# nnaisense/evotorch

Hardware: NVIDIA H100
Metric: PGPE generations/sec at popsize=1Mxdim=10k (Rastrigin, fp32) (higher is better)
Workload: dtype f32

## Files before the change

evotorch_b200/csrc/evok_grad.cu:

```cuda
#include <dlfcn.h>

#include <atomic>
#include <cstdlib>

#include "evok_common.cuh"

#ifndef EVOK_GRAD_TMA_DEFAULT
#define EVOK_GRAD_TMA_DEFAULT 1
#endif

namespace evok {

constexpr int kGradThreads = 256;
constexpr int kGradUnroll = 4;
constexpr int kGradMinBlocks = 4;
constexpr int kGradCtasPerSm = 4;
constexpr int kMaxResidentCtas = kNumSMs * 8;

template <int VEC>
struct VecF;
template <>
struct VecF<4> {
  float v[4];
};
template <>
struct VecF<1> {
  float v[1];
};

template <int VEC>
__device__ __forceinline__ VecF<VEC> load_row(const float* p) {
  VecF<VEC> r;
  if (VEC == 4) {
    const float4 t = ld_stream4(p);
    r.v[0] = t.x; r.v[1] = t.y; r.v[2] = t.z; r.v[3] = t.w;
  } else {
    r.v[0] = ld_stream1(p);
  }
  return r;
}

struct GradItems {
  int64_t x, w, mu, sigma, partial;
};

struct SepWeights {
  const float* q;
  int active;
  float* wsum_partial;
};

constexpr int kEpsRead = 0, kEpsRegen = 1, kEpsRebuild = 2;

__device__ __forceinline__ void grad_coeffs(int form, float s, float& c1, float& c0) {
  if (form == EVOK_GRAD_EXP) {
    c1 = __fdiv_rn(1.0f, s * s);
    c0 = 1.0f;
  } else if (form == EVOK_GRAD_MOMENTS) {
    c1 = 1.0f;
    c0 = 0.0f;
  } else {
    c1 = __fdiv_rn(1.0f, s);
    c0 = s;
  }
}

template <bool SYM, bool SEPW = false>
__device__ __forceinline__ void row_weights(const float* __restrict__ w, int64_t r, float& a, float& b, int64_t D = 0,
                                            const SepWeights* sepw = nullptr) {
  if (SEPW) {
    const float aw = __ldg(w + r);
    a = fmaxf(aw, 0.0f);
    b = (sepw->active && aw < 0.0f) ? __fdiv_rn((float)D * aw, __ldg(sepw->q + r)) : aw;
  } else if (SYM) {
    const float wp = __ldg(w + 2 * r), wm = __ldg(w + 2 * r + 1);
    a = 0.5f * (wp - wm);
    b = 0.5f * (wp + wm);
  } else {
    a = b = __ldg(w + r);
  }
}

__device__ __forceinline__ void accumulate(float a, float b, float e, float c1, float c0, float& s1, float& s2) {
  s1 = fmaf(a, e, s1);
  s2 = fmaf(b, fmaf(e * e, c1, -c0), s2);
}

template <int VEC, bool TAIL = true>
__device__ __forceinline__ void store_partial(float* partial, int64_t chunk, int64_t D, int64_t col, const float* s1, const float* s2) {
  float* p1 = partial + (chunk * 2 + 0) * D + col;
  float* p2 = partial + (chunk * 2 + 1) * D + col;
#pragma unroll
  for (int c = 0; c < VEC; ++c) {
    if (!TAIL || col + c < D) {
      p1[c] = s1[c];
      p2[c] = s2[c];
    }
  }
}

template <int VEC, int TX, bool SYM, int EPS, bool SEPW = false>
__global__ void __launch_bounds__(kGradThreads, kGradMinBlocks)
    grad_partial_kernel(int form, const float* __restrict__ X, int64_t ldx, const float* __restrict__ w, const float* __restrict__ mu,
                        const float* __restrict__ sigma, int64_t n_units, int64_t D, int64_t units_per_chunk, uint64_t unit0,
                        const __grid_constant__ PhiloxKey key, const uint32_t* __restrict__ stream_off, float* __restrict__ partial,
                        const __grid_constant__ GradItems items, const __grid_constant__ SepWeights sepw) {
  static_assert(!SEPW || (EPS == kEpsRegen && !SYM), "the CMA-ES weight mode regenerates non-symmetric rows");
  constexpr int TY = kGradThreads / TX;
  if (gridDim.z > 1) {
    const int64_t item = blockIdx.z;
    X += item * items.x;
    w += item * items.w;
    mu += item * items.mu;
    sigma += item * items.sigma;
    partial += item * items.partial;
  }
  const uint32_t sw = key.stream_lo + ((EPS != kEpsRead && stream_off) ? __ldg(stream_off) : 0u) + (EPS == kEpsRebuild ? (uint32_t)blockIdx.z : 0u);
  const int tx = threadIdx.x % TX, ty = threadIdx.x / TX;
  const int64_t col = ((int64_t)blockIdx.x * TX + tx) * VEC;
  const bool active = col < D;

  float m[VEC], c1[VEC], c0[VEC], sg[VEC];
#pragma unroll
  for (int c = 0; c < VEC; ++c) {
    const bool ok = active && (col + c < D) && !SEPW;
    const float s = ok ? __ldg(sigma + col + c) : 1.0f;
    m[c] = ok ? __ldg(mu + col + c) : 0.0f;
    sg[c] = s;
    grad_coeffs(form, s, c1[c], c0[c]);
  }

  float s1[VEC], s2[VEC];
#pragma unroll
  for (int c = 0; c < VEC; ++c) s1[c] = s2[c] = 0.0f;

  const int64_t r_begin = (int64_t)blockIdx.y * units_per_chunk;
  const int64_t r_end = min(n_units, r_begin + units_per_chunk);
  float wb = 0.0f;

  for (int64_t r0 = r_begin + ty; r0 < r_end; r0 += (int64_t)TY * kGradUnroll) {
    float a[kGradUnroll], b[kGradUnroll];
    bool need[kGradUnroll];
    VecF<VEC> x[kGradUnroll];
#pragma unroll
    for (int u = 0; u < kGradUnroll; ++u) {
      const int64_t r = r0 + (int64_t)u * TY;
      a[u] = b[u] = 0.0f;
      if (r < r_end) {
        row_weights<SYM, SEPW>(w, r, a[u], b[u], D, &sepw);
        if (SEPW) wb += b[u];
      }
      need[u] = active && (a[u] != 0.0f || b[u] != 0.0f);
    }
#pragma unroll
    for (int u = 0; u < kGradUnroll; ++u) {
      const int64_t r = r0 + (int64_t)u * TY;
      if (need[u]) {
        if (EPS != kEpsRead) {
          if (VEC == 4) {
            normals4(key, sw, unit0 + (uint64_t)r, (uint32_t)(col >> 2), x[u].v);
          } else {
            float z[4];
            normals4(key, sw, unit0 + (uint64_t)r, (uint32_t)(col >> 2), z);
            x[u].v[0] = z[col & 3];
          }
        } else {
          x[u] = load_row<VEC>(X + (SYM ? 2 * r : r) * ldx + col);
        }
      }
    }
#pragma unroll
    for (int u = 0; u < kGradUnroll; ++u) {
      if (need[u]) {
#pragma unroll
        for (int c = 0; c < VEC; ++c) {
          const float e = EPS == kEpsRegen ? sg[c] * x[u].v[c] : EPS == kEpsRebuild ? fmaf(sg[c], x[u].v[c], m[c]) - m[c] : x[u].v[c] - m[c];
          accumulate(a[u], b[u], e, c1[c], c0[c], s1[c], s2[c]);
        }
      }
    }
  }

  __shared__ float red[TY > 1 ? TY : 1][TX][2 * VEC];
  if (TY > 1) {
#pragma unroll
    for (int c = 0; c < VEC; ++c) {
      red[ty][tx][c] = s1[c];
      red[ty][tx][VEC + c] = s2[c];
    }
    __syncthreads();
    if (ty == 0) {
#pragma unroll
      for (int c = 0; c < VEC; ++c) {
        float t1 = red[0][tx][c], t2 = red[0][tx][VEC + c];
        for (int y = 1; y < TY; ++y) {
          t1 += red[y][tx][c];
          t2 += red[y][tx][VEC + c];
        }
        s1[c] = t1;
        s2[c] = t2;
      }
    }
  }
  if (ty == 0 && active) store_partial<VEC>(partial, blockIdx.y, D, col, s1, s2);
  if (SEPW && blockIdx.x == 0) {
    __shared__ float wred[TY];
    if (tx == 0) wred[ty] = wb;
    __syncthreads();
    if (threadIdx.x == 0) {
      float t = wred[0];
      for (int y = 1; y < TY; ++y) t += wred[y];
      sepw.wsum_partial[blockIdx.y] = t;
    }
  }
}

__device__ __forceinline__ void sum_chunks(const float* __restrict__ partial, int n_chunks, int64_t D, int64_t j, float& t1, float& t2) {
  t1 = 0.0f;
  t2 = 0.0f;
  for (int c = 0; c < n_chunks; ++c) {
    t1 += partial[((int64_t)c * 2 + 0) * D + j];
    t2 += partial[((int64_t)c * 2 + 1) * D + j];
  }
}

template <bool WSUM = false>
__global__ void __launch_bounds__(256) grad_finalize_kernel(const float* __restrict__ partial, int n_chunks, int64_t D, float scale_mu,
                                                            float scale_sigma, float* __restrict__ out_mu, float* __restrict__ out_sigma,
                                                            int64_t item_stride_partial = 0, const float* __restrict__ wsum_partial = nullptr,
                                                            float* __restrict__ wsum_out = nullptr) {
  const int64_t j = (int64_t)blockIdx.x * blockDim.x + threadIdx.x;
  if (WSUM && j == 0) {
    float t = 0.0f;
    for (int c = 0; c < n_chunks; ++c) t += wsum_partial[c];
    *wsum_out = t;
  }
  if (j >= D) return;
  partial += (int64_t)blockIdx.y * item_stride_partial;
  out_mu += (int64_t)blockIdx.y * D;
  out_sigma += (int64_t)blockIdx.y * D;
  float t1, t2;
  sum_chunks(partial, n_chunks, D, j, t1, t2);
  out_mu[j] = t1 * scale_mu;
  out_sigma[j] = t2 * scale_sigma;
}

struct GradPush {
  PeerSink sink;
  const unsigned long long* epoch;
  unsigned int* done;
};

__global__ void __launch_bounds__(256) grad_finalize_push_kernel(const float* __restrict__ partial, int n_chunks, int64_t D, float scale_mu,
                                                                 float scale_sigma, const __grid_constant__ PeerSink sink,
                                                                 const unsigned long long* epoch, unsigned int* done) {
  const int64_t j = (int64_t)blockIdx.x * blockDim.x + threadIdx.x;
  if (j < D) {
    float t1, t2;
    sum_chunks(partial, n_chunks, D, j, t1, t2);
    t1 *= scale_mu;
    t2 *= scale_sigma;
    for (int p = 0; p < sink.world; ++p) {
      float* slot = static_cast<float*>(sink.data[p]) + (int64_t)sink.rank * 2 * D;
      slot[j] = t1;
      slot[D + j] = t2;
    }
  }
  peer_signal_tail(sink, epoch, done);
}

#ifndef EVOK_GRAD_TMA_ROWS
#define EVOK_GRAD_TMA_ROWS 4
#endif
#ifndef EVOK_GRAD_TMA_STAGES
#define EVOK_GRAD_TMA_STAGES 4
#endif
#ifndef EVOK_GRAD_TMA_CTAS_PER_SM
#define EVOK_GRAD_TMA_CTAS_PER_SM 3
#endif
constexpr int kTmaRows = EVOK_GRAD_TMA_ROWS;
constexpr int kTmaStages = EVOK_GRAD_TMA_STAGES;
constexpr int kTmaCols = 1024;
constexpr int kTmaConsumers = 256;
constexpr int kTmaThreads = kTmaConsumers + 32;
constexpr size_t kTmaSmemBytes = (size_t)kTmaStages * kTmaRows * kTmaCols * sizeof(float) + 2 * kTmaStages * sizeof(uint64_t) + 128;

__device__ __forceinline__ uint32_t smem_u32(const void* p) { return (uint32_t)__cvta_generic_to_shared(p); }
__device__ __forceinline__ void mbar_init(uint64_t* bar, uint32_t count) {
  asm volatile("mbarrier.init.shared::cta.b64 [%0], %1;" ::"r"(smem_u32(bar)), "r"(count) : "memory");
}
__device__ __forceinline__ void mbar_expect_tx(uint64_t* bar, uint32_t bytes) {
  asm volatile("mbarrier.arrive.expect_tx.shared::cta.b64 _, [%0], %1;" ::"r"(smem_u32(bar)), "r"(bytes) : "memory");
}
__device__ __forceinline__ void mbar_arrive(uint64_t* bar) {
  asm volatile("mbarrier.arrive.shared::cta.b64 _, [%0];" ::"r"(smem_u32(bar)) : "memory");
}
__device__ __forceinline__ void mbar_wait(uint64_t* bar, uint32_t parity) {
  asm volatile(
      "{\n"
      ".reg .pred P1;\n"
      "LAB_WAIT:\n"
      "mbarrier.try_wait.parity.shared::cta.b64 P1, [%0], %1;\n"
      "@P1 bra DONE;\n"
      "bra LAB_WAIT;\n"
      "DONE:\n"
      "}" ::"r"(smem_u32(bar)), "r"(parity) : "memory");
}
__device__ __forceinline__ void bulk_load(void* dst_smem, const void* src_gmem, uint32_t bytes, uint64_t* bar) {
  asm volatile("cp.async.bulk.shared::cluster.global.mbarrier::complete_tx::bytes [%0], [%1], %2, [%3];" ::"r"(smem_u32(dst_smem)),
               "l"(src_gmem), "r"(bytes), "r"(smem_u32(bar))
               : "memory");
}

constexpr int kSplitPeriod = 16;
__device__ __forceinline__ uint32_t rebuilt_mask(int split) {
  uint32_t m = 0;
#pragma unroll
  for (int k = 0; k < kSplitPeriod; ++k)
    if ((k + 1) * split / kSplitPeriod > k * split / kSplitPeriod) m |= 1u << k;
  return m;
}
__device__ __forceinline__ bool group_rebuilt(uint32_t mask, int64_t g) { return (mask >> ((int)g & (kSplitPeriod - 1))) & 1u; }

template <bool SYM>
__global__ void __launch_bounds__(kTmaThreads, EVOK_GRAD_TMA_CTAS_PER_SM)
    grad_partial_tma_kernel(int form, const float* __restrict__ X, int64_t ldx, const float* __restrict__ w, const float* __restrict__ mu,
                            const float* __restrict__ sigma, int64_t n_units, int64_t D, int64_t units_per_chunk, int split, uint64_t unit0,
                            const __grid_constant__ PhiloxKey key, const uint32_t* __restrict__ stream_off, float* __restrict__ partial) {
  extern __shared__ __align__(128) unsigned char smem_raw[];
  float* tiles = reinterpret_cast<float*>(smem_raw);
  uint64_t* full = reinterpret_cast<uint64_t*>(smem_raw + (size_t)kTmaStages * kTmaRows * kTmaCols * sizeof(float));
  uint64_t* empty = full + kTmaStages;

  const int tid = threadIdx.x, warp = tid >> 5, lane = tid & 31;
  const int64_t col0 = (int64_t)blockIdx.x * kTmaCols;
  const int64_t width = min((int64_t)kTmaCols, D - col0);
  const int64_t r_begin = (int64_t)blockIdx.y * units_per_chunk;
  const int64_t r_end = min(n_units, r_begin + units_per_chunk);
  const int64_t n_rows = r_end - r_begin;
  const int64_t n_groups = (n_rows + kTmaRows - 1) / kTmaRows;
  const int64_t row_stride = (SYM ? 2 : 1) * ldx;
  const uint32_t mask = rebuilt_mask(split);

  if (tid == 0) {
    for (int s = 0; s < kTmaStages; ++s) {
      mbar_init(&full[s], 1);
      mbar_init(&empty[s], kTmaConsumers / 32);
    }
    asm volatile("fence.mbarrier_init.release.cluster;" ::: "memory");
  }
  __syncthreads();

  if (warp == kTmaConsumers / 32) {
    if (lane == 0) {
      const uint32_t row_bytes = (uint32_t)(width * sizeof(float));
      int64_t t = 0;
      for (int64_t g = 0; g < n_groups; ++g) {
        if (group_rebuilt(mask, g)) continue;
        const int s = (int)(t % kTmaStages);
        const uint32_t use = (uint32_t)(t / kTmaStages);
        ++t;
        if (use > 0) mbar_wait(&empty[s], (use - 1) & 1);
        const int64_t r0 = r_begin + g * kTmaRows;
        const int rows = (int)min((int64_t)kTmaRows, r_end - r0);
        mbar_expect_tx(&full[s], rows * row_bytes);
        float* dst = tiles + (size_t)s * kTmaRows * kTmaCols;
        for (int i = 0; i < rows; ++i) bulk_load(dst + (size_t)i * kTmaCols, X + (r0 + i) * row_stride + col0, row_bytes, &full[s]);
      }
    }
    return;
  }

  const int64_t col = col0 + (int64_t)tid * 4;
  const bool active = col < D;
  const uint32_t sw = key.stream_lo + (stream_off ? __ldg(stream_off) : 0u);
  const int frm = SYM ? EVOK_GRAD_SYMMETRIC : form;
  float m[4], sg[4], c1[4], c0[4];
#pragma unroll
  for (int c = 0; c < 4; ++c) {
    sg[c] = active ? __ldg(sigma + col + c) : 1.0f;
    m[c] = active ? __ldg(mu + col + c) : 0.0f;
    grad_coeffs(frm, sg[c], c1[c], c0[c]);
  }
  float s1[4] = {0.f, 0.f, 0.f, 0.f}, s2[4] = {0.f, 0.f, 0.f, 0.f};

  int64_t t = 0;
  for (int64_t g = 0; g < n_groups; ++g) {
    const int64_t r0 = r_begin + g * kTmaRows;
    const int rows = (int)min((int64_t)kTmaRows, r_end - r0);
    float a[kTmaRows], b[kTmaRows];
    bool need[kTmaRows];
#pragma unroll
    for (int i = 0; i < kTmaRows; ++i) {
      a[i] = b[i] = 0.0f;
      if (i < rows) row_weights<SYM>(w, r0 + i, a[i], b[i]);
      need[i] = a[i] != 0.0f || b[i] != 0.0f;
    }
    if (group_rebuilt(mask, g)) {
      if (active) {
        float x[kTmaRows][4];
#pragma unroll
        for (int i = 0; i < kTmaRows; ++i) {
          float z[4];
          normals4(key, sw, unit0 + (uint64_t)(r0 + i), (uint32_t)(col >> 2), z);
#pragma unroll
          for (int c = 0; c < 4; ++c) x[i][c] = fmaf(sg[c], z[c], m[c]);
        }
#pragma unroll
        for (int i = 0; i < kTmaRows; ++i) {
          if (need[i]) {
#pragma unroll
            for (int c = 0; c < 4; ++c) accumulate(a[i], b[i], x[i][c] - m[c], c1[c], c0[c], s1[c], s2[c]);
          }
        }
      }
      continue;
    }
    const int s = (int)(t % kTmaStages);
    const uint32_t use = (uint32_t)(t / kTmaStages);
    ++t;
    mbar_wait(&full[s], use & 1);
    const float4* tile = reinterpret_cast<const float4*>(tiles + (size_t)s * kTmaRows * kTmaCols) + tid;
    if (active) {
      float4 v4[kTmaRows];
#pragma unroll
      for (int i = 0; i < kTmaRows; ++i) v4[i] = tile[(size_t)i * (kTmaCols / 4)];
#pragma unroll
      for (int i = 0; i < kTmaRows; ++i) {
        if (need[i]) {
          const float4 v = v4[i];
          const float x[4] = {v.x, v.y, v.z, v.w};
#pragma unroll
          for (int c = 0; c < 4; ++c) accumulate(a[i], b[i], x[c] - m[c], c1[c], c0[c], s1[c], s2[c]);
        }
      }
    }
    __syncwarp();
    if (lane == 0) mbar_arrive(&empty[s]);
  }
  if (active) store_partial<4, false>(partial, blockIdx.y, D, col, s1, s2);
}

constexpr int kAutoSplitCapped = 2;
constexpr int kAutoSplitFull = 5;
constexpr int64_t kFullPowerMilliwatts = 550000;

static int auto_split_for_power(int64_t milliwatts) { return milliwatts >= kFullPowerMilliwatts ? kAutoSplitFull : kAutoSplitCapped; }

static int64_t enforced_power_limit_mw(int device) {
  char bus_id[32];
  if (cudaDeviceGetPCIBusId(bus_id, (int)sizeof(bus_id), device) != cudaSuccess) {
    cudaGetLastError();
    return -1;
  }
  void* nvml = dlopen("libnvidia-ml.so.1", RTLD_NOW | RTLD_LOCAL);
  if (!nvml) return -1;
  using init_t = int (*)();
  using by_bus_t = int (*)(const char*, void**);
  using limit_t = int (*)(void*, unsigned int*);
  const auto init = reinterpret_cast<init_t>(dlsym(nvml, "nvmlInit_v2"));
  const auto shutdown = reinterpret_cast<init_t>(dlsym(nvml, "nvmlShutdown"));
  const auto by_bus = reinterpret_cast<by_bus_t>(dlsym(nvml, "nvmlDeviceGetHandleByPciBusId_v2"));
  const auto limit = reinterpret_cast<limit_t>(dlsym(nvml, "nvmlDeviceGetEnforcedPowerLimit"));
  int64_t mw = -1;
  if (init && shutdown && by_bus && limit && init() == 0) {
    void* handle = nullptr;
    unsigned int v = 0;
    if (by_bus(bus_id, &handle) == 0 && limit(handle, &v) == 0) mw = v;
    shutdown();
  }
  dlclose(nvml);
  return mw;
}

static int device_auto_split() {
  constexpr int kMaxDevices = 64;
  static std::atomic<int> resolved[kMaxDevices];
  int device = 0;
  if (cudaGetDevice(&device) != cudaSuccess || device < 0 || device >= kMaxDevices) {
    cudaGetLastError();
    return kAutoSplitCapped;
  }
  int s = resolved[device].load(std::memory_order_relaxed);
  if (s == 0) {
    s = auto_split_for_power(enforced_power_limit_mw(device)) + 1;
    resolved[device].store(s, std::memory_order_relaxed);
  }
  return s - 1;
}


struct GradCall {
  GradCall(int form, int eps, const float* w, const float* mu, const float* sigma, int64_t n_rows, int64_t D, float scale_mu, float scale_sigma,
           float* out_mu, float* out_sigma, void* ws, size_t ws_bytes, void* stream)
      : form(form), eps(eps), w(w), mu(mu), sigma(sigma), n_rows(n_rows), D(D), scale_mu(scale_mu), scale_sigma(scale_sigma), out_mu(out_mu),
        out_sigma(out_sigma), ws(ws), ws_bytes(ws_bytes), st((cudaStream_t)stream) {}
  int form;
  int eps;
  const float* w;
  const float* mu;
  const float* sigma;
  int64_t n_rows, D;
  float scale_mu, scale_sigma;
  float* out_mu;
  float* out_sigma;
  void* ws;
  size_t ws_bytes;
  cudaStream_t st;
  const float* X = nullptr;
  int64_t ldx = 0;
  int64_t row0 = 0;
  PhiloxKey key{};
  const uint32_t* stream_off = nullptr;
  bool batched = false;
  int64_t n_items = 1;
  GradItems items{0, 0, 0, 0, 0};
  int split = 0;
  SepWeights sepw{nullptr, 0, nullptr};
  float* wsum = nullptr;
  const GradPush* push = nullptr;
};

static bool is_sym(const GradCall& c) { return c.form == EVOK_GRAD_SYMMETRIC; }

struct GradPlan {
  bool tma;
  int vec, tx, n_coltiles, n_chunks;
  int64_t n_units, units_per_chunk;
};

static void set_chunks(GradPlan& p, int64_t chunks) {
  if (chunks < 1) chunks = 1;
  if (chunks > 65535) chunks = 65535;
  p.units_per_chunk = (p.n_units + chunks - 1) / chunks;
  p.n_chunks = (int)((p.n_units + p.units_per_chunk - 1) / p.units_per_chunk);
}

static bool tma_enabled() {
  const char* env = getenv("EVOK_GRAD_TMA");
  return env ? atoi(env) != 0 : EVOK_GRAD_TMA_DEFAULT != 0;
}

static GradPlan plan_grad(const GradCall& c) {
  GradPlan p{};
  p.n_units = is_sym(c) ? c.n_rows / 2 : c.n_rows;
  const bool vec_ok = c.eps == kEpsRegen || (c.D % 4 == 0 && (c.eps == kEpsRebuild || (c.ldx % 4 == 0 && aligned16(c.X) && c.items.x % 4 == 0)) &&
                                             c.items.mu % 4 == 0 && c.items.sigma % 4 == 0);
  p.vec = vec_ok ? 4 : 1;
  p.tma = !c.batched && c.eps == kEpsRead && vec_ok && c.form != EVOK_GRAD_MOMENTS && c.D >= 512 && p.n_units >= 4096 && tma_enabled();
  if (p.tma) {
    p.n_coltiles = (int)((c.D + kTmaCols - 1) / kTmaCols);
    set_chunks(p, (int64_t)kNumSMs * EVOK_GRAD_TMA_CTAS_PER_SM / p.n_coltiles);
    return p;
  }
  const int64_t col_threads = (c.D + p.vec - 1) / p.vec;
  p.tx = 32;
  while (p.tx < kGradThreads && p.tx < col_threads) p.tx <<= 1;
  p.n_coltiles = (int)((col_threads + p.tx - 1) / p.tx);
  const int ty = kGradThreads / p.tx;
  int64_t chunks = (int64_t)kNumSMs * kGradCtasPerSm / p.n_coltiles;
  const int64_t max_useful = (p.n_units + (int64_t)ty * kGradUnroll * 16 - 1) / ((int64_t)ty * kGradUnroll * 16);
  set_chunks(p, chunks < max_useful ? chunks : max_useful);
  chunks = ((int64_t)kNumSMs * kGradCtasPerSm + (int64_t)p.n_coltiles * c.n_items - 1) / ((int64_t)p.n_coltiles * c.n_items);
  if (chunks < p.n_chunks) set_chunks(p, chunks);
  if (c.eps == kEpsRebuild && !vec_ok) {
    p.vec = 4;
    p.n_coltiles = (int)(((c.D + 3) / 4 + p.tx - 1) / p.tx);
  }
  return p;
}

using PartialKernel = void (*)(int, const float*, int64_t, const float*, const float*, const float*, int64_t, int64_t, int64_t, uint64_t,
                               PhiloxKey, const uint32_t*, float*, GradItems, SepWeights);
#define EVOK_GRAD_TXS(VEC, SYM, EPS, SEPW)                                                                             \
  {                                                                                                                    \
    grad_partial_kernel<VEC, 32, SYM, EPS, SEPW>, grad_partial_kernel<VEC, 64, SYM, EPS, SEPW>,                        \
        grad_partial_kernel<VEC, 128, SYM, EPS, SEPW>, grad_partial_kernel<VEC, 256, SYM, EPS, SEPW>                   \
  }
static const PartialKernel kPartialKernels[9][4] = {
    EVOK_GRAD_TXS(1, false, kEpsRead, false),    EVOK_GRAD_TXS(1, true, kEpsRead, false),  EVOK_GRAD_TXS(4, false, kEpsRead, false),
    EVOK_GRAD_TXS(4, true, kEpsRead, false),     EVOK_GRAD_TXS(4, false, kEpsRegen, false), EVOK_GRAD_TXS(4, true, kEpsRegen, false),
    EVOK_GRAD_TXS(4, false, kEpsRebuild, false), EVOK_GRAD_TXS(4, true, kEpsRebuild, false), EVOK_GRAD_TXS(4, false, kEpsRegen, true)};
#undef EVOK_GRAD_TXS

static int partial_row(int eps, int vec, bool sym, bool sepw) { return sepw ? 8 : 2 * (eps == kEpsRead ? vec / 4 : 1 + eps) + (sym ? 1 : 0); }
static int tx_index(int tx) { return tx == 32 ? 0 : tx == 64 ? 1 : tx == 128 ? 2 : 3; }

static void launch_partial(const GradCall& c, const GradPlan& p, int64_t b0, int64_t nb, float* partial) {
  PhiloxKey key = c.key;
  key.stream_lo += (uint32_t)b0;
  const float* X = c.X + b0 * c.items.x;
  const float* w = c.w + b0 * c.items.w;
  const float* mu = c.mu + b0 * c.items.mu;
  const float* sigma = c.sigma + b0 * c.items.sigma;
  const uint64_t unit0 = (uint64_t)(is_sym(c) ? c.row0 / 2 : c.row0);
  if (p.tma) {
    const int rebuilt = c.split < 0 ? device_auto_split() : c.split;
    auto kernel = is_sym(c) ? grad_partial_tma_kernel<true> : grad_partial_tma_kernel<false>;
    cudaFuncSetAttribute(kernel, cudaFuncAttributeMaxDynamicSharedMemorySize, (int)kTmaSmemBytes);
    kernel<<<dim3(p.n_coltiles, p.n_chunks), kTmaThreads, kTmaSmemBytes, c.st>>>(c.form, X, c.ldx, w, mu, sigma, p.n_units, c.D, p.units_per_chunk,
                                                                                  rebuilt, unit0, key, c.stream_off, partial);
    return;
  }
  const PartialKernel kernel = kPartialKernels[partial_row(c.eps, p.vec, is_sym(c), c.wsum != nullptr)][tx_index(p.tx)];
  kernel<<<dim3(p.n_coltiles, p.n_chunks, (unsigned)nb), kGradThreads, 0, c.st>>>(c.form, X, c.ldx, w, mu, sigma, p.n_units, c.D,
                                                                                    p.units_per_chunk, unit0, key, c.stream_off, partial, c.items, c.sepw);
}

static int launch_finalize(const GradCall& c, int n_chunks, int64_t b0, int64_t nb, const float* partial) {
  const unsigned grid = (unsigned)((c.D + 255) / 256);
  if (c.push) {
    grad_finalize_push_kernel<<<grid, 256, 0, c.st>>>(partial, n_chunks, c.D, c.scale_mu, c.scale_sigma, c.push->sink, c.push->epoch, c.push->done);
  } else if (c.wsum) {
    grad_finalize_kernel<true><<<grid, 256, 0, c.st>>>(partial, n_chunks, c.D, c.scale_mu, c.scale_sigma, c.out_mu, c.out_sigma, 0, c.sepw.wsum_partial,
                                                       c.wsum);
  } else {
    grad_finalize_kernel<<<dim3(grid, (unsigned)nb), 256, 0, c.st>>>(partial, n_chunks, c.D, c.scale_mu, c.scale_sigma, c.out_mu + b0 * c.D,
                                                                     c.out_sigma + b0 * c.D, c.items.partial);
  }
  EVOK_CHECK_LAUNCH();
  return 0;
}

static int run_grad(GradCall c) {
  if (c.n_items == 0) return 0;
  float* partial = (float*)c.ws;
  if ((is_sym(c) ? c.n_rows / 2 : c.n_rows) == 0) {
    if (c.push) return launch_finalize(c, 0, 0, 1, partial);
    cudaMemsetAsync(c.out_mu, 0, (size_t)c.n_items * c.D * 4, c.st);
    cudaMemsetAsync(c.out_sigma, 0, (size_t)c.n_items * c.D * 4, c.st);
    return 0;
  }
  const GradPlan p = plan_grad(c);
  c.items.partial = (int64_t)p.n_chunks * 2 * c.D;
  const int64_t chunk = c.n_items < kMaxGridY ? c.n_items : kMaxGridY;
  if (c.ws_bytes < (size_t)chunk * c.items.partial * sizeof(float)) return EVOK_E_WORKSPACE;
  return for_item_chunks(c.n_items, kMaxGridY, [&](int64_t b0, int64_t nb) {
    launch_partial(c, p, b0, nb, partial);
    EVOK_CHECK_LAUNCH();
    return launch_finalize(c, p.n_chunks, b0, nb, partial);
  });
}

static bool bad_form(int form) { return form < EVOK_GRAD_SEPARABLE || form > EVOK_GRAD_MOMENTS; }

static int grad_single(const GradCall& c) {
  const bool read = c.eps == kEpsRead;
  if ((!c.w && c.n_rows != 0) || !c.mu || !c.sigma || !c.ws || (read && !c.X) || (!c.push && (!c.out_mu || !c.out_sigma))) return EVOK_E_NULLPTR;
  if (bad_form(c.form)) return EVOK_E_BADENUM;
  if (c.n_rows < 0 || c.D <= 0 || c.row0 < 0 || (read && c.ldx < c.D) || c.split < -1 || c.split > kSplitPeriod) return EVOK_E_BADSIZE;
  if (is_sym(c) && ((c.n_rows & 1) || (c.row0 & 1))) return EVOK_E_ODDROWS;
  if (c.ws_bytes < evok_grad_workspace_bytes(c.n_rows, c.D)) return EVOK_E_WORKSPACE;
  return run_grad(c);
}

static int grad_batched(const GradCall& c) {
  const bool read = c.eps == kEpsRead;
  if ((read && !c.X) || !c.w || !c.mu || !c.sigma || !c.out_mu || !c.out_sigma || !c.ws) return EVOK_E_NULLPTR;
  if (bad_form(c.form)) return EVOK_E_BADENUM;
  if (c.n_items < 0 || c.n_rows < 0 || c.D <= 0 || (read && c.ldx < c.D) || c.items.x < 0 || c.items.mu < 0 || c.items.sigma < 0)
    return EVOK_E_BADSIZE;
  if (is_sym(c) && (c.n_rows & 1)) return EVOK_E_ODDROWS;
  return run_grad(c);
}

}

using namespace evok;

extern "C" EVOK_API size_t evok_grad_workspace_bytes(int64_t n_rows, int64_t D) {
  (void)n_rows;
  if (D <= 0) return 256;
  return ((size_t)kMaxResidentCtas * 1024 + 2 * (size_t)D + 64) * sizeof(float);
}

extern "C" EVOK_API int evok_grad(int form, const float* X, int64_t ldx, const float* w, const float* mu, const float* sigma, int64_t n_rows,
                         int64_t D, float scale_mu, float scale_sigma, float* out_mu, float* out_sigma, void* ws, size_t ws_bytes,
                         void* stream) {
  GradCall c(form, kEpsRead, w, mu, sigma, n_rows, D, scale_mu, scale_sigma, out_mu, out_sigma, ws, ws_bytes, stream);
  c.X = X;
  c.ldx = ldx;
  return grad_single(c);
}

extern "C" EVOK_API int evok_grad_regen(int form, const float* w, const float* mu, const float* sigma, int64_t row0, int64_t n_rows, int64_t D,
                               uint64_t seed, uint64_t stream_id, const uint32_t* stream_offset_dev, float scale_mu, float scale_sigma,
                               float* out_mu, float* out_sigma, void* ws, size_t ws_bytes, void* stream) {
  GradCall c(form, kEpsRegen, w, mu, sigma, n_rows, D, scale_mu, scale_sigma, out_mu, out_sigma, ws, ws_bytes, stream);
  c.row0 = row0;
  c.key = make_philox_key(seed, stream_id);
  c.stream_off = stream_offset_dev;
  return grad_single(c);
}

extern "C" EVOK_API int evok_grad_hybrid(int form, const float* X, int64_t ldx, const float* w, const float* mu, const float* sigma, int64_t row0,
                                         int64_t n_rows, int64_t D, uint64_t seed, uint64_t stream_id, const uint32_t* stream_offset_dev, int split,
                                         float scale_mu, float scale_sigma, float* out_mu, float* out_sigma, void* ws, size_t ws_bytes, void* stream) {
  GradCall c(form, kEpsRead, w, mu, sigma, n_rows, D, scale_mu, scale_sigma, out_mu, out_sigma, ws, ws_bytes, stream);
  c.X = X;
  c.ldx = ldx;
  c.row0 = row0;
  c.key = make_philox_key(seed, stream_id);
  c.stream_off = stream_offset_dev;
  c.split = split;
  return grad_single(c);
}

extern "C" EVOK_API int evok_grad_auto_split(int64_t power_limit_mw) { return auto_split_for_power(power_limit_mw); }

extern "C" EVOK_API int64_t evok_grad_power_limit_mw(int device) { return enforced_power_limit_mw(device); }

extern "C" EVOK_API size_t evok_sepcma_workspace_bytes(int64_t n_rows, int64_t D) {
  return evok_grad_workspace_bytes(n_rows, D) + (size_t)kMaxResidentCtas * sizeof(float);
}

extern "C" EVOK_API int evok_sepcma_moments(const float* aw, const float* q, int active, int64_t row0, int64_t n_rows, int64_t D, uint64_t seed,
                                            uint64_t stream_id, const uint32_t* stream_offset_dev, float* local, float* S2, float* wsum, void* ws,
                                            size_t ws_bytes, void* stream) {
  if (!aw || (active && !q) || !local || !S2 || !wsum || !ws) return EVOK_E_NULLPTR;
  if (n_rows <= 0 || D <= 0 || row0 < 0) return EVOK_E_BADSIZE;
  if (ws_bytes < evok_sepcma_workspace_bytes(n_rows, D)) return EVOK_E_WORKSPACE;
  GradCall c(EVOK_GRAD_MOMENTS, kEpsRegen, aw, nullptr, nullptr, n_rows, D, 1.0f, 1.0f, local, S2, ws, ws_bytes, stream);
  c.row0 = row0;
  c.key = make_philox_key(seed, stream_id);
  c.stream_off = stream_offset_dev;
  c.sepw = SepWeights{q, active, (float*)ws + evok_grad_workspace_bytes(n_rows, D) / sizeof(float)};
  c.wsum = wsum;
  return run_grad(c);
}

extern "C" EVOK_API int evok_grad_push(int form, const float* X, int64_t ldx, const float* w, const float* mu, const float* sigma, int64_t row0,
                                       int64_t n_rows, int64_t D, uint64_t seed, uint64_t stream_id, const uint32_t* stream_offset_dev,
                                       float scale_mu, float scale_sigma, int world, int rank, void* const* peer_slots, void* const* peer_flags,
                                       const uint64_t* epoch_dev, uint32_t* done_dev, void* ws, size_t ws_bytes, void* stream) {
  if (!peer_slots || !peer_flags || !epoch_dev || !done_dev) return EVOK_E_NULLPTR;
  if (world < 1 || world > EVOK_MAX_PEERS || rank < 0 || rank >= world) return EVOK_E_BADSIZE;
  GradPush push{};
  push.sink.world = world;
  push.sink.rank = rank;
  for (int p = 0; p < world; ++p) {
    if (!peer_slots[p] || !peer_flags[p]) return EVOK_E_NULLPTR;
    push.sink.data[p] = peer_slots[p];
    push.sink.flags[p] = static_cast<unsigned long long*>(peer_flags[p]);
  }
  push.epoch = reinterpret_cast<const unsigned long long*>(epoch_dev);
  push.done = done_dev;
  GradCall c(form, X ? kEpsRead : kEpsRegen, w, mu, sigma, n_rows, D, scale_mu, scale_sigma, nullptr, nullptr, ws, ws_bytes, stream);
  c.X = X;
  c.ldx = X ? ldx : 0;
  c.row0 = row0;
  c.key = make_philox_key(seed, stream_id);
  c.stream_off = stream_offset_dev;
  c.push = &push;
  return grad_single(c);
}

extern "C" EVOK_API size_t evok_grad_batched_workspace_bytes(int64_t n_items, int64_t n_rows, int64_t D) {
  if (n_items <= 0 || D <= 0) return 256;
  (void)n_rows;
  return ((size_t)kMaxResidentCtas * 1024 + 4 * (size_t)n_items * (size_t)D + 64) * sizeof(float);
}

extern "C" EVOK_API int evok_grad_batched(int form, const float* X, int64_t item_stride_x, int64_t ldx, const float* w, const float* mu,
                                          int64_t item_stride_mu, const float* sigma, int64_t item_stride_sigma, int64_t n_items, int64_t n_rows,
                                          int64_t D, float scale_mu, float scale_sigma, float* out_mu, float* out_sigma, void* ws, size_t ws_bytes,
                                          void* stream) {
  GradCall c(form, kEpsRead, w, mu, sigma, n_rows, D, scale_mu, scale_sigma, out_mu, out_sigma, ws, ws_bytes, stream);
  c.X = X;
  c.ldx = ldx;
  c.batched = true;
  c.n_items = n_items;
  c.items = GradItems{item_stride_x, n_rows, item_stride_mu, item_stride_sigma, 0};
  return grad_batched(c);
}

extern "C" EVOK_API int evok_grad_batched_regen(int form, const float* w, const float* mu, int64_t item_stride_mu, const float* sigma,
                                                int64_t item_stride_sigma, int64_t n_items, int64_t n_rows, int64_t D, uint64_t seed,
                                                uint64_t stream_id0, float scale_mu, float scale_sigma, float* out_mu, float* out_sigma, void* ws,
                                                size_t ws_bytes, void* stream) {
  GradCall c(form, kEpsRebuild, w, mu, sigma, n_rows, D, scale_mu, scale_sigma, out_mu, out_sigma, ws, ws_bytes, stream);
  c.key = make_philox_key(seed, stream_id0);
  c.batched = true;
  c.n_items = n_items;
  c.items = GradItems{0, n_rows, item_stride_mu, item_stride_sigma, 0};
  return grad_batched(c);
}
```

Baseline: 55.73.

## Stage per-row fitness weights in a shared-memory ring filled by the producer warp

Before this change, every consumer thread computed row_weights from global memory for each group of rows. Now the producer warp loads a batch of up to 32 rows' weights (one lane per row) into a triple-buffered shared-memory ring, guarded by new full/empty mbarriers. Consumers read the weights from that ring instead of global memory. The aim is to take redundant global weight loads and weight math off the consumer critical path. The cost is a little more shared memory, extra barrier handshakes, and the producer warp now running all 32 lanes instead of only lane 0.

```diff
diff --git a/evotorch_b200/csrc/evok_grad.cu b/evotorch_b200/csrc/evok_grad.cu
--- a/evotorch_b200/csrc/evok_grad.cu
+++ b/evotorch_b200/csrc/evok_grad.cu
@@ -283,7 +283,16 @@
 constexpr int kTmaCols = 1024;
 constexpr int kTmaConsumers = 256;
 constexpr int kTmaThreads = kTmaConsumers + 32;
-constexpr size_t kTmaSmemBytes = (size_t)kTmaStages * kTmaRows * kTmaCols * sizeof(float) + 2 * kTmaStages * sizeof(uint64_t) + 128;
+constexpr int kWeightGroups = 32 / kTmaRows > 0 ? 32 / kTmaRows : 1;
+constexpr int kWeightRows = kWeightGroups * kTmaRows;
+constexpr int kWeightSlots = 3;
+static_assert(kWeightRows <= 32, "one producer lane per row of a weight batch");
+struct __align__(16) GroupWeights {
+  float a[kTmaRows], b[kTmaRows];
+};
+constexpr size_t kTmaTileBytes = (size_t)kTmaStages * kTmaRows * kTmaCols * sizeof(float);
+constexpr size_t kTmaWeightBytes = (size_t)kWeightSlots * kWeightGroups * sizeof(GroupWeights);
+constexpr size_t kTmaSmemBytes = kTmaTileBytes + kTmaWeightBytes + 2 * (kTmaStages + kWeightSlots) * sizeof(uint64_t) + 128;
 
 __device__ __forceinline__ uint32_t smem_u32(const void* p) { return (uint32_t)__cvta_generic_to_shared(p); }
 __device__ __forceinline__ void mbar_init(uint64_t* bar, uint32_t count) {
@@ -329,8 +338,11 @@
                             const __grid_constant__ PhiloxKey key, const uint32_t* __restrict__ stream_off, float* __restrict__ partial) {
   extern __shared__ __align__(128) unsigned char smem_raw[];
   float* tiles = reinterpret_cast<float*>(smem_raw);
-  uint64_t* full = reinterpret_cast<uint64_t*>(smem_raw + (size_t)kTmaStages * kTmaRows * kTmaCols * sizeof(float));
+  GroupWeights* wring = reinterpret_cast<GroupWeights*>(smem_raw + kTmaTileBytes);
+  uint64_t* full = reinterpret_cast<uint64_t*>(smem_raw + kTmaTileBytes + kTmaWeightBytes);
   uint64_t* empty = full + kTmaStages;
+  uint64_t* wfull = empty + kTmaStages;
+  uint64_t* wempty = wfull + kWeightSlots;
 
   const int tid = threadIdx.x, warp = tid >> 5, lane = tid & 31;
   const int64_t col0 = (int64_t)blockIdx.x * kTmaCols;
@@ -339,6 +351,7 @@
   const int64_t r_end = min(n_units, r_begin + units_per_chunk);
   const int64_t n_rows = r_end - r_begin;
   const int64_t n_groups = (n_rows + kTmaRows - 1) / kTmaRows;
+  const int64_t n_batches = (n_groups + kWeightGroups - 1) / kWeightGroups;
   const int64_t row_stride = (SYM ? 2 : 1) * ldx;
   const uint32_t mask = rebuilt_mask(split);
 
@@ -347,26 +360,50 @@
       mbar_init(&full[s], 1);
       mbar_init(&empty[s], kTmaConsumers / 32);
     }
+    for (int k = 0; k < kWeightSlots; ++k) {
+      mbar_init(&wfull[k], 32);
+      mbar_init(&wempty[k], kTmaConsumers / 32);
+    }
     asm volatile("fence.mbarrier_init.release.cluster;" ::: "memory");
   }
   __syncthreads();
 
   if (warp == kTmaConsumers / 32) {
-    if (lane == 0) {
-      const uint32_t row_bytes = (uint32_t)(width * sizeof(float));
-      int64_t t = 0;
-      for (int64_t g = 0; g < n_groups; ++g) {
-        if (group_rebuilt(mask, g)) continue;
-        const int s = (int)(t % kTmaStages);
-        const uint32_t use = (uint32_t)(t / kTmaStages);
-        ++t;
-        if (use > 0) mbar_wait(&empty[s], (use - 1) & 1);
-        const int64_t r0 = r_begin + g * kTmaRows;
-        const int rows = (int)min((int64_t)kTmaRows, r_end - r0);
-        mbar_expect_tx(&full[s], rows * row_bytes);
-        float* dst = tiles + (size_t)s * kTmaRows * kTmaCols;
-        for (int i = 0; i < rows; ++i) bulk_load(dst + (size_t)i * kTmaCols, X + (r0 + i) * row_stride + col0, row_bytes, &full[s]);
+    auto stage_weights = [&](int64_t j) {
+      const int k = (int)(j % kWeightSlots);
+      const uint32_t use = (uint32_t)(j / kWeightSlots);
+      if (use > 0) mbar_wait(&wempty[k], (use - 1) & 1);
+      if (lane < kWeightRows) {
+        const int64_t r = r_begin + j * kWeightRows + lane;
+        float a = 0.0f, b = 0.0f;
+        if (r < r_end) row_weights<SYM>(w, r, a, b);
+        GroupWeights& gw = wring[k * kWeightGroups + lane / kTmaRows];
+        gw.a[lane % kTmaRows] = a;
+        gw.b[lane % kTmaRows] = b;
       }
+      mbar_arrive(&wfull[k]);
+    };
+    const uint32_t row_bytes = (uint32_t)(width * sizeof(float));
+    int64_t t = 0;
+    stage_weights(0);
+    for (int64_t j = 0; j < n_batches; ++j) {
+      if (j + 1 < n_batches) stage_weights(j + 1);
+      if (lane == 0) {
+        const int64_t g_end = min(n_groups, (j + 1) * kWeightGroups);
+        for (int64_t g = j * kWeightGroups; g < g_end; ++g) {
+          if (group_rebuilt(mask, g)) continue;
+          const int s = (int)(t % kTmaStages);
+          const uint32_t use = (uint32_t)(t / kTmaStages);
+          ++t;
+          if (use > 0) mbar_wait(&empty[s], (use - 1) & 1);
+          const int64_t r0 = r_begin + g * kTmaRows;
+          const int rows = (int)min((int64_t)kTmaRows, r_end - r0);
+          mbar_expect_tx(&full[s], rows * row_bytes);
+          float* dst = tiles + (size_t)s * kTmaRows * kTmaCols;
+          for (int i = 0; i < rows; ++i) bulk_load(dst + (size_t)i * kTmaCols, X + (r0 + i) * row_stride + col0, row_bytes, &full[s]);
+        }
+      }
+      __syncwarp();
     }
     return;
   }
@@ -385,16 +422,30 @@
   float s1[4] = {0.f, 0.f, 0.f, 0.f}, s2[4] = {0.f, 0.f, 0.f, 0.f};
 
   int64_t t = 0;
+  int gb = 0, k = 0;
+  uint32_t wphase = 0;
   for (int64_t g = 0; g < n_groups; ++g) {
     const int64_t r0 = r_begin + g * kTmaRows;
-    const int rows = (int)min((int64_t)kTmaRows, r_end - r0);
+    if (gb == 0) mbar_wait(&wfull[k], wphase);
+    const GroupWeights gw = wring[k * kWeightGroups + gb];
     float a[kTmaRows], b[kTmaRows];
     bool need[kTmaRows];
 #pragma unroll
     for (int i = 0; i < kTmaRows; ++i) {
-      a[i] = b[i] = 0.0f;
-      if (i < rows) row_weights<SYM>(w, r0 + i, a[i], b[i]);
+      a[i] = gw.a[i];
+      b[i] = gw.b[i];
       need[i] = a[i] != 0.0f || b[i] != 0.0f;
+    }
+    if (gb == kWeightGroups - 1 || g == n_groups - 1) {
+      __syncwarp();
+      if (lane == 0) mbar_arrive(&wempty[k]);
+    }
+    if (++gb == kWeightGroups) {
+      gb = 0;
+      if (++k == kWeightSlots) {
+        k = 0;
+        wphase ^= 1u;
+      }
     }
     if (group_rebuilt(mask, g)) {
       if (active) {
```

Measured after the change: 56.25 (median of 6 runs). No clear change (+0.9%).
